# kennethsoh/IE-ACHE

Measured on AMD Instinct MI355X. Metric: bootstrapped gate ops/sec; encrypted 32-bit MUL/sec, higher is better.
Workload: dtype int32; 1 GPU; 16-bit ADD, batch 4096 ciphertext pairs, 1xMI355X (level-batched bootstraps); circuit=add16, batch_per_gpu=4096, bootstraps_per_expr=80, levels=48, params=n=630 N=1024 k=1 l=3 Bgbit=7 ks_t=8 ks_basebit=2, parallelism=batch-sharded x1, kernel=w1x64-radix8-onelimb, overlap_streams=2, rccl_ranks=0

## Files before the change

ie-ache_amd/csrc/blind_rotate_w64.hip:

```cpp
#include "blind_rotate_w64.h"

#include <cstdio>
#include <algorithm>
#include <stdexcept>
#include <type_traits>
#include <vector>

#include "br_step.h"
#include "mix_plan.h"

namespace ieache {
namespace w64 {

using namespace dev;

namespace {

__global__ __launch_bounds__(64) void k_bk_to_spectrum_w64(const Torus32* bk_raw, double2* bkf) {
    __shared__ __align__(16) double2 sT[kTile];
    __shared__ __align__(16) double2 sTw[kTwElems];
    const int lane = threadIdx.x;
    build_twiddles(sTw, lane, 64);
    __syncthreads();
    const LaneRoots R = make_roots(sTw, lane);
    const size_t poly = blockIdx.x;
    const Torus32* src = bk_raw + poly * kN;
    const size_t irow = poly >> 1, c = poly & 1;
#pragma unroll 1
    for (int limb = 0; limb < 2; limb++) {
        double2 x[8];
#pragma unroll
        for (int r = 0; r < 8; r++) {
            const int32_t v0 = src[64 * r + lane], v1 = src[64 * r + lane + kM];
            const int32_t lo0 = (int16_t)(v0 & 0xFFFF), lo1 = (int16_t)(v1 & 0xFFFF);
            const int32_t e0 = limb ? (int32_t)(((int64_t)v0 - lo0) >> 16) : lo0;
            const int32_t e1 = limb ? (int32_t)(((int64_t)v1 - lo1) >> 16) : lo1;
            x[r] = make_double2((double)e0, (double)e1);
        }
        fft512_forward<true>(x, sT, lane, R);
        double2* dst = bkf + ((irow * 4 + c * 2 + limb) * 8) * 64 + lane;
#pragma unroll
        for (int k2 = 0; k2 < 8; k2++) dst[k2 * 64] = x[k2];
    }
}

__global__ __launch_bounds__(64) void k_bk_to_spectrum_w64_1(const Torus32* bk_raw, double2* bkf1) {
    __shared__ __align__(16) double2 sT[kTile];
    __shared__ __align__(16) double2 sTw[kTwElems];
    const int lane = threadIdx.x;
    build_twiddles(sTw, lane, 64);
    __syncthreads();
    const LaneRoots R = make_roots(sTw, lane);
    const size_t poly = blockIdx.x;
    const Torus32* src = bk_raw + poly * kN;
    double2 x[8];
#pragma unroll
    for (int r = 0; r < 8; r++) {
        const double2 v = make_double2((double)src[64 * r + lane], (double)src[64 * r + lane + kM]);
        x[r] = v;
    }
    fft512_forward<true>(x, sT, lane, R);
    double2* dst = bkf1 + (poly * 8) * 64 + lane;
#pragma unroll
    for (int k2 = 0; k2 < 8; k2++) dst[k2 * 64] = x[k2];
}

template <bool TV>
__global__ __launch_bounds__(128) void k_br_prologue(DevKeys K, WorkDesc W, uint16_t* st_bara, int32_t nb, int32_t* st_acc) {
    __shared__ int32_t s_barb;
    const int tid = threadIdx.x;
    const int32_t n = K.n;
    const int64_t item = (int64_t)blockIdx.x;
    const GateInst g = resolve(W, W.item0 + item, K.stride);
    uint16_t* bara = st_bara + (size_t)item * nb;
    for (int32_t i = tid; i <= n; i += 128) {
        const int32_t bar = modswitch2N(combined_coef(g, i, n), 11);
        if (i < n)
            bara[i] = (uint16_t)bar;
        else
            s_barb = bar;
    }
    __syncthreads();
    const int32_t a0 = (2 * kN - s_barb) & (2 * kN - 1);
    int32_t* acc = st_acc + (size_t)item * 2 * kN;
    const Torus32* v = TV ? test_poly_row(W, W.item0 + item, kN) : nullptr;
#pragma unroll
    for (int r = 0; r < 8; r++) {
        const int32_t j = 128 * r + tid;
        acc[j] = 0;
        if (TV)
            acc[kN + j] = rot_coef(v, j, a0, kN);
        else
            acc[kN + j] = ((j - a0) & (2 * kN - 1)) < kN ? kMU : -kMU;
    }
}

template <int L, int BGBIT, int XLANE = 1>
__global__ __launch_bounds__(128, 2) void k_blind_rotate_w2(DevKeys K, const double2* __restrict__ bkf,
                                                           const uint16_t* __restrict__ st_bara, int32_t nb,
                                                           int32_t* st_acc, int32_t i0, int32_t i1, Torus32* ext,
                                                           const double2* __restrict__ gtw) {
    extern __shared__ __align__(16) unsigned char smem[];
    double2* sT_all = reinterpret_cast<double2*>(smem);
    double2* sTw = sT_all + 2 * kTile;
    int32_t* acc = reinterpret_cast<int32_t*>(sTw + kTwElems);
    const int tid = threadIdx.x, lane = tid & 63, wave = tid >> 6;
    double2* sT = sT_all + wave * kTile;
    const double2* sTp = sT_all + (wave ^ 1) * kTile;
    const int64_t item = (int64_t)blockIdx.x;
    const uint16_t* __restrict__ bara = st_bara + (size_t)item * nb;
    int32_t* gacc = st_acc + (size_t)item * 2 * kN;
    load_twiddles(sTw, gtw, tid, 128);
    const LaneRoots R = make_roots(sTw, lane);
    copy_acc<128>(acc, gacc, tid);
    __syncthreads();

    uint32_t dec_offset = decomposition_offset<L, BGBIT>();
    int32_t* accw = acc + wave * kN;

    const int32_t my_a = lane_amounts(bara, i0, i1, lane);
#pragma unroll 1
    for (int32_t i = i0; i < i1; i++) {
        const int32_t a = __builtin_amdgcn_readlane(my_a, i - i0);
        if (a == 0) continue;
        const double2* __restrict__ bki = bkf + (size_t)i * (2 * L * 4 * kM) + (size_t)(2 * wave) * kM + lane;
        double2 s[2][8];
        uint32_t v0[8], v1[8];
#pragma unroll
        for (int r = 0; r < 8; r++) {
            const int32_t j = 64 * r + lane;
            v0[r] = (((uint32_t)rot_coef(accw, j, a, kN) - (uint32_t)accw[j]) + dec_offset) ^ dec_offset;
            v1[r] = (((uint32_t)rot_coef(accw, j + kM, a, kN) - (uint32_t)accw[j + kM]) + dec_offset) ^ dec_offset;
        }
        auto digit_row = [&](const int q, auto first) {
            constexpr bool FIRST = decltype(first)::value;
            const int sh = 32 - (q + 1) * BGBIT;
            const double2* __restrict__ bown = bki + (size_t)(wave * L + q) * (4 * kM);
            const double2* __restrict__ bpar = bki + (size_t)((wave ^ 1) * L + q) * (4 * kM);
            double2 x[8];
            digits_to_double2<BGBIT>(x, v0, v1, sh);
            double2 bA[8], bB[8], bC[8];
#pragma unroll
            for (int k = 0; k < 8; k++) bA[k] = bown[k * 64];
            __builtin_amdgcn_sched_barrier(0);
            fft512_forward<true, XLANE>(x, sT, lane, R);
#pragma unroll
            for (int k = 0; k < 8; k++) sT[k * 64 + lane] = x[k];
#pragma unroll
            for (int k = 0; k < 8; k++) bB[k] = bown[(8 + k) * 64];
#pragma unroll
            for (int k = 0; k < 8; k++) bC[k] = bpar[k * 64];
            __builtin_amdgcn_sched_barrier(0);
            mac_row<FIRST>(s[0], x, bA);
            __builtin_amdgcn_sched_barrier(0);
#pragma unroll
            for (int k = 0; k < 8; k++) bA[k] = bpar[(8 + k) * 64];
            __builtin_amdgcn_sched_barrier(0);
            mac_row<FIRST>(s[1], x, bB);
            __syncthreads();
#pragma unroll
            for (int k = 0; k < 8; k++) x[k] = sTp[k * 64 + lane];
            mac_row<false>(s[0], x, bC);
            mac_row<false>(s[1], x, bA);
            __syncthreads();
        };
        digit_row(0, std::true_type{});
#pragma unroll 1
        for (int q = 1; q < L; q++) digit_row(q, std::false_type{});
        fft512_inverse_pair<true>(s[0], s[1], sT, lane, R);
#pragma unroll
        for (int r = 0; r < 8; r++) {
            double unused = 0.0;
            const uint32_t l0 = round_coef(s[0][r].x, untwist_gain(r), false, unused), l1 = round_coef(s[0][r].y, untwist_gain(r), false, unused);
            const uint32_t h0 = round_coef(s[1][r].x, untwist_gain(r), false, unused), h1 = round_coef(s[1][r].y, untwist_gain(r), false, unused);
            const int32_t j = 64 * r + lane;
            accw[j] = (int32_t)((uint32_t)accw[j] + l0 + (h0 << 16));
            accw[j + kM] = (int32_t)((uint32_t)accw[j + kM] + l1 + (h1 << 16));
        }
    }
    __syncthreads();
    finish_slice<128>(ext, item, acc, gacc, tid);
}


template <int L, int BGBIT, int GUARD, bool DIAG = false, int G = kW1Gates>
__global__ __launch_bounds__(64 * G, 2) void k_blind_rotate_w1b(DevKeys K, const double2* __restrict__ bkf1,
                                                                       const uint16_t* __restrict__ st_bara, int32_t nb,
                                                                       int32_t* st_acc, int64_t items, int32_t i0, int32_t i1,
                                                                       Torus32* ext, unsigned* guard,
                                                                       const double2* __restrict__ gtw, unsigned long long* diag = nullptr) {
    extern __shared__ __align__(16) unsigned char smem[];
    int32_t* acc_all = reinterpret_cast<int32_t*>(smem);
    double2* sT_all = reinterpret_cast<double2*>(smem + (size_t)G * 2 * kN * 4);
    double2* sTw = sT_all + G * kTile;
    const int tid = threadIdx.x, lane = tid & 63;
    const int wave = __builtin_amdgcn_readfirstlane(tid >> 6);
    double2* sT = sT_all + wave * kTile;
    int32_t* acc = acc_all + wave * 2 * kN;
    const int64_t item = (int64_t)blockIdx.x * G + wave;
    load_twiddles(sTw, gtw, tid, 64 * G);
    __syncthreads();
    if (item >= items) return;
    const LaneRoots R = make_roots(sTw, lane);
    const uint16_t* __restrict__ bara = st_bara + (size_t)item * nb;
    int32_t* gacc = st_acc + (size_t)item * 2 * kN;
    {
        const int4* src = reinterpret_cast<const int4*>(gacc);
        int4* dst = reinterpret_cast<int4*>(acc);
#pragma unroll
        for (int r = 0; r < 8; r++) dst[64 * r + lane] = src[64 * r + lane];
    }
    wave_sync();

    constexpr uint32_t halfBg = 1u << (BGBIT - 1);
    uint32_t dec_offset = 0;
#pragma unroll
    for (int q = 1; q <= L; q++) dec_offset += halfBg << (32 - q * BGBIT);
    double dev_max = 0.0;
    constexpr int kRowBytes = 2 * kM * (int)sizeof(double2), kStepBytes = 2 * L * kRowBytes;
    const __amdgpu_buffer_rsrc_t bk_rsrc = bk_resource(bkf1, K.n, kStepBytes);
    const int lane16 = bk_lane_offset(lane);
    const unsigned char* accb = reinterpret_cast<const unsigned char*>(acc_all);
    const uint32_t pb0 = (uint32_t)wave * (2 * kN * 4);

    unsigned long long tsum[8] = {0, 0, 0, 0, 0, 0, 0, 0}, tlast = 0;
    if (DIAG) tlast = stamp();
    const int32_t my_a = lane_amounts(bara, i0, i1, lane);
#pragma unroll 1
    for (int32_t i = i0; i < i1; i++) {
        const int32_t a = __builtin_amdgcn_readlane(my_a, i - i0);
        if (a == 0) continue;
        const int bki = i * kStepBytes;
        double2 s[2][8];
        uint32_t v0[8], v1[8];
        const uint32_t jb4 = ((uint32_t)(lane - a) & (2 * kN - 1)) << 2;
        auto decompose = [&](const uint32_t pb) {
            const int32_t* accp = reinterpret_cast<const int32_t*>(accb + pb);
            decompose_rotated(v0, v1, accb, accp, pb, jb4, lane, dec_offset);
        };
        auto digit_row = [&](const int sh, const int brow, auto first) {
            constexpr bool FIRST = decltype(first)::value;
            double2 x[8], bA[8], bB[8];
            load_bk_block(bA, bk_rsrc, lane16, brow);
            digits_to_double2<BGBIT>(x, v0, v1, sh);
            __builtin_amdgcn_sched_barrier(0);
            stamp_phase<DIAG>(tsum, tlast, 1);
            fft512_forward<true, 1>(x, sT, lane, R);
            stamp_phase<DIAG>(tsum, tlast, 2);
            load_bk_block(bB, bk_rsrc, lane16, brow + kRowBytes / 2);
            __builtin_amdgcn_sched_barrier(0);
#pragma unroll
            for (int k = 0; k < 8; k++) s[0][k] = mac<FIRST>(s[0][k], x[k], bA[k]);
#pragma unroll
            for (int k = 0; k < 8; k++) s[1][k] = mac<FIRST>(s[1][k], x[k], bB[k]);
            stamp_phase<DIAG>(tsum, tlast, 3);
        };
        decompose(pb0);
        stamp_phase<DIAG>(tsum, tlast, 0);
        digit_row(32 - BGBIT, bki, std::true_type{});
#pragma unroll 1
        for (int row = 1; row < L; row++) digit_row(32 - (row + 1) * BGBIT, bki + row * kRowBytes, std::false_type{});
        decompose(pb0 + 4096u);
        stamp_phase<DIAG>(tsum, tlast, 0);
#pragma unroll 1
        for (int row = L; row < 2 * L; row++) digit_row(32 - (row - L + 1) * BGBIT, bki + row * kRowBytes, std::false_type{});
        fft512_inverse_pair<true>(s[0], s[1], sT, lane, R);
        stamp_phase<DIAG>(tsum, tlast, 4);
#pragma unroll
        for (int c = 0; c < 2; c++) {
            uint32_t* accc = reinterpret_cast<uint32_t*>(acc) + c * kN;
#pragma unroll
            for (int r = 0; r < 8; r++) {
                const bool watched = GUARD == 1 || (GUARD == 2 && (r & 3) == 0);
                const uint32_t d0 = round_coef(s[c][r].x, untwist_gain(r), watched, dev_max), d1 = round_coef(s[c][r].y, untwist_gain(r), watched, dev_max);
                const int32_t j = 64 * r + lane;
                __hip_atomic_fetch_add(&accc[j], d0, __ATOMIC_RELAXED, __HIP_MEMORY_SCOPE_WAVEFRONT);
                __hip_atomic_fetch_add(&accc[j + kM], d1, __ATOMIC_RELAXED, __HIP_MEMORY_SCOPE_WAVEFRONT);
            }
        }
        wave_sync();
        stamp_phase<DIAG>(tsum, tlast, 5);
    }
    if (DIAG && diag && lane == 0) {
#pragma unroll
        for (int t = 0; t < 8; t++) atomicAdd(&diag[(wave & 1) * 8 + t], tsum[t]);
    }
    if (GUARD) publish_guard(dev_max, guard, lane);
    finish_slice<64>(ext, item, acc, gacc, lane);
}

template <int L, int BGBIT, int G = kW1Gates>
__global__ __launch_bounds__(64 * G, 2) void k_blind_rotate_x1(DevKeys K, const double2* __restrict__ bkf,
                                                                      const uint16_t* __restrict__ st_bara, int32_t nb,
                                                                      int32_t* st_acc, int64_t items, int32_t i0, int32_t i1,
                                                                      Torus32* ext, const double2* __restrict__ gtw) {
    extern __shared__ __align__(16) unsigned char smem[];
    int32_t* acc_all = reinterpret_cast<int32_t*>(smem);
    double2* sT_all = reinterpret_cast<double2*>(smem + (size_t)G * 2 * kN * 4);
    double2* sTw = sT_all + G * kTile;
    const int tid = threadIdx.x, lane = tid & 63;
    const int wave = __builtin_amdgcn_readfirstlane(tid >> 6);
    double2* sT = sT_all + wave * kTile;
    int32_t* acc = acc_all + wave * 2 * kN;
    const int64_t item = (int64_t)blockIdx.x * G + wave;
    load_twiddles(sTw, gtw, tid, 64 * G);
    __syncthreads();
    if (item >= items) return;
    const LaneRoots R = make_roots(sTw, lane);
    const uint16_t* __restrict__ bara = st_bara + (size_t)item * nb;
    int32_t* gacc = st_acc + (size_t)item * 2 * kN;
    {
        const int4* src = reinterpret_cast<const int4*>(gacc);
        int4* dst = reinterpret_cast<int4*>(acc);
#pragma unroll
        for (int r = 0; r < 8; r++) dst[64 * r + lane] = src[64 * r + lane];
    }
    wave_sync();

    constexpr uint32_t halfBg = 1u << (BGBIT - 1);
    uint32_t dec_offset = 0;
#pragma unroll
    for (int q = 1; q <= L; q++) dec_offset += halfBg << (32 - q * BGBIT);
    constexpr int kBlockBytes = kM * (int)sizeof(double2), kRowBytes = 4 * kBlockBytes, kStepBytes = 2 * L * kRowBytes;
    const __amdgpu_buffer_rsrc_t bk_rsrc = bk_resource(bkf, K.n, kStepBytes);
    const int lane16 = bk_lane_offset(lane);
    const unsigned char* accb = reinterpret_cast<const unsigned char*>(acc_all);
    const uint32_t pb0 = (uint32_t)wave * (2 * kN * 4);

    const int32_t my_a = lane_amounts(bara, i0, i1, lane);
#pragma unroll 1
    for (int32_t i = i0; i < i1; i++) {
        const int32_t a = __builtin_amdgcn_readlane(my_a, i - i0);
        if (a == 0) continue;
        const int bki = i * kStepBytes;
        double2 s[4][8];
        uint32_t v0[8], v1[8];
        const uint32_t jb4 = ((uint32_t)(lane - a) & (2 * kN - 1)) << 2;
        auto decompose = [&](const uint32_t pb, const uint32_t jb) {
            const int32_t* accp = reinterpret_cast<const int32_t*>(accb + pb);
            decompose_rotated(v0, v1, accb, accp, pb, jb, lane, dec_offset);
        };
        auto digit_row = [&](const int sh, const int brow, auto first) {
            constexpr bool FIRST = decltype(first)::value;
            double2 x[8], bA[8], bB[8];
            digits_to_double2<BGBIT>(x, v0, v1, sh);
            __builtin_amdgcn_sched_barrier(0);
            auto req = [&]() { load_bk_block(bA, bk_rsrc, lane16, brow); };
            fft512_forward<true, 1, decltype(req), true>(x, sT, lane, R, req);
            load_bk_block(bB, bk_rsrc, lane16, brow + kBlockBytes);
            __builtin_amdgcn_sched_barrier(0);
            mac_row<FIRST>(s[0], x, bA);
            __builtin_amdgcn_sched_barrier(0);
            load_bk_block(bA, bk_rsrc, lane16, brow + 2 * kBlockBytes);
            __builtin_amdgcn_sched_barrier(0);
            mac_row<FIRST>(s[1], x, bB);
            __builtin_amdgcn_sched_barrier(0);
            load_bk_block(bB, bk_rsrc, lane16, brow + 3 * kBlockBytes);
            __builtin_amdgcn_sched_barrier(0);
            mac_row<FIRST>(s[2], x, bA);
            mac_row<FIRST>(s[3], x, bB);
        };
        decompose(pb0, jb4);
        digit_row(32 - BGBIT, bki, std::true_type{});
#pragma unroll 1
        for (int row = 1; row < L; row++) digit_row(32 - (row + 1) * BGBIT, bki + row * kRowBytes, std::false_type{});
        uint32_t jb4b = jb4;
        asm volatile("" : "+v"(jb4b));
        decompose(pb0 + 4096u, jb4b);
#pragma unroll 1
        for (int row = L; row < 2 * L; row++) digit_row(32 - (row - L + 1) * BGBIT, bki + row * kRowBytes, std::false_type{});
#pragma unroll
        for (int c = 0; c < 2; c++) {
            fft512_inverse_pair<true>(s[2 * c], s[2 * c + 1], sT, lane, R);
            uint32_t* accc = reinterpret_cast<uint32_t*>(acc) + c * kN;
#pragma unroll
            for (int r = 0; r < 8; r++) {
                double unused = 0.0;
                const uint32_t d0 = round_coef(s[2 * c][r].x, untwist_gain(r), false, unused) + (round_coef(s[2 * c + 1][r].x, untwist_gain(r), false, unused) << 16);
                const uint32_t d1 = round_coef(s[2 * c][r].y, untwist_gain(r), false, unused) + (round_coef(s[2 * c + 1][r].y, untwist_gain(r), false, unused) << 16);
                const int32_t j = 64 * r + lane;
                __hip_atomic_fetch_add(&accc[j], d0, __ATOMIC_RELAXED, __HIP_MEMORY_SCOPE_WAVEFRONT);
                __hip_atomic_fetch_add(&accc[j + kM], d1, __ATOMIC_RELAXED, __HIP_MEMORY_SCOPE_WAVEFRONT);
            }
        }
        wave_sync();
    }
    finish_slice<64>(ext, item, acc, gacc, lane);
}

template <int L, int BGBIT, int GUARD>
__global__ __launch_bounds__(128, 2) void k_blind_rotate_w2r(DevKeys K, const double2* __restrict__ bkf1,
                                                            const uint16_t* __restrict__ st_bara, int32_t nb,
                                                            int32_t* st_acc, int32_t i0, int32_t i1, Torus32* ext,
                                                            unsigned* guard, const double2* __restrict__ gtw) {
    extern __shared__ __align__(16) unsigned char smem[];
    int32_t* acc = reinterpret_cast<int32_t*>(smem);
    double2* sT_all = reinterpret_cast<double2*>(smem + (size_t)2 * kN * 4);
    double2* sTw = sT_all + 2 * kTile;
    const int tid = threadIdx.x, lane = tid & 63;
    const int wave = __builtin_amdgcn_readfirstlane(tid >> 6);
    double2* sT = sT_all + wave * kTile;
    const double2* sTp = sT_all + (wave ^ 1) * kTile;
    const int64_t item = (int64_t)blockIdx.x;
    const uint16_t* __restrict__ bara = st_bara + (size_t)item * nb;
    int32_t* gacc = st_acc + (size_t)item * 2 * kN;
    load_twiddles(sTw, gtw, tid, 128);
    const LaneRoots R = make_roots(sTw, lane);
    {
        const int4* src = reinterpret_cast<const int4*>(gacc);
        int4* dst = reinterpret_cast<int4*>(acc);
#pragma unroll
        for (int r = 0; r < 4; r++) dst[128 * r + tid] = src[128 * r + tid];
    }
    __syncthreads();

    constexpr uint32_t halfBg = 1u << (BGBIT - 1);
    uint32_t dec_offset = 0;
#pragma unroll
    for (int q = 1; q <= L; q++) dec_offset += halfBg << (32 - q * BGBIT);
    double dev_max = 0.0;
    constexpr int kRowBytes = 2 * kM * (int)sizeof(double2), kStepBytes = 2 * L * kRowBytes;
    const __amdgpu_buffer_rsrc_t bk_rsrc = bk_resource(bkf1, K.n, kStepBytes);
    const int lane16 = bk_lane_offset(lane);
    const unsigned char* accb = reinterpret_cast<const unsigned char*>(acc);
    const uint32_t pb = (uint32_t)wave * (kN * 4);
    const int32_t* accp = acc + wave * kN;
    uint32_t* accu = reinterpret_cast<uint32_t*>(acc) + wave * kN;

    int32_t my_a = 0;
#pragma unroll 1
    for (int32_t i = i0; i < i1; i++) {
        if (((i - i0) & 63) == 0) my_a = (i + lane < i1) ? (int32_t)bara[i + lane] : 0;
        const int32_t a = __builtin_amdgcn_readlane(my_a, (i - i0) & 63);
        if (a == 0) continue;
        const int bki = i * kStepBytes + wave * L * kRowBytes;
        double2 s[2][8];
        uint32_t v0[8], v1[8];
        const uint32_t jb4 = ((uint32_t)(lane - a) & (2 * kN - 1)) << 2;
#pragma unroll
        for (int r = 0; r < 8; r++) {
            const uint32_t t = jb4 + 256u * r;
            const uint32_t o0 = (t & 4092u) | pb, o1 = o0 ^ 2048u;
            const int32_t m0 = __builtin_amdgcn_sbfe((int32_t)t, 12, 1), m1 = __builtin_amdgcn_sbfe((int32_t)(t + 2048u), 12, 1);
            const uint32_t rv0 = *reinterpret_cast<const uint32_t*>(accb + o0), rv1 = *reinterpret_cast<const uint32_t*>(accb + o1);
            const uint32_t pv0 = (uint32_t)accp[64 * r + lane], pv1 = (uint32_t)accp[64 * r + lane + kM];
            v0[r] = ((rv0 ^ (uint32_t)m0) + ((dec_offset - pv0) - (uint32_t)m0)) ^ dec_offset;
            v1[r] = ((rv1 ^ (uint32_t)m1) + ((dec_offset - pv1) - (uint32_t)m1)) ^ dec_offset;
        }
        auto digit_row = [&](const int sh, const int brow, auto first) {
            constexpr bool FIRST = decltype(first)::value;
            double2 x[8], bA[8], bB[8];
            load_bk_block(bA, bk_rsrc, lane16, brow);
            digits_to_double2<BGBIT>(x, v0, v1, sh);
            __builtin_amdgcn_sched_barrier(0);
            fft512_forward<true, 1>(x, sT, lane, R);
            load_bk_block(bB, bk_rsrc, lane16, brow + kRowBytes / 2);
            __builtin_amdgcn_sched_barrier(0);
#pragma unroll
            for (int k = 0; k < 8; k++) s[0][k] = mac<FIRST>(s[0][k], x[k], bA[k]);
#pragma unroll
            for (int k = 0; k < 8; k++) s[1][k] = mac<FIRST>(s[1][k], x[k], bB[k]);
        };
        digit_row(32 - BGBIT, bki, std::true_type{});
#pragma unroll 1
        for (int q = 1; q < L; q++) digit_row(32 - (q + 1) * BGBIT, bki + q * kRowBytes, std::false_type{});
        double2 y[8];
#pragma unroll
        for (int k = 0; k < 8; k++) {
            const double2 mine = wave ? s[1][k] : s[0][k], theirs = wave ? s[0][k] : s[1][k];
            sT[k * 64 + lane] = theirs;
            y[k] = mine;
        }
        __syncthreads();
#pragma unroll
        for (int k = 0; k < 8; k++) {
            const double2 z = sTp[k * 64 + lane];
            y[k] = cadd(y[k], z);
        }
        __syncthreads();
        fft512_inverse<true>(y, sT, lane, R);
#pragma unroll
        for (int r = 0; r < 8; r++) {
            const bool watched = GUARD == 1 || (GUARD == 2 && (r & 3) == 0);
            const uint32_t d0 = round_coef(y[r].x, untwist_gain(r), watched, dev_max), d1 = round_coef(y[r].y, untwist_gain(r), watched, dev_max);
            const int32_t j = 64 * r + lane;
            __hip_atomic_fetch_add(&accu[j], d0, __ATOMIC_RELAXED, __HIP_MEMORY_SCOPE_WAVEFRONT);
            __hip_atomic_fetch_add(&accu[j + kM], d1, __ATOMIC_RELAXED, __HIP_MEMORY_SCOPE_WAVEFRONT);
        }
        wave_sync();
    }
    __syncthreads();
    if (GUARD) publish_guard(dev_max, guard, lane);
    finish_slice<128>(ext, item, acc, gacc, tid);
}

template <int L, int BGBIT, int GUARD>
__global__ __launch_bounds__(256, 2) void k_blind_rotate_w4r(DevKeys K, const double2* __restrict__ bkf1,
                                                            const uint16_t* __restrict__ st_bara, int32_t nb,
                                                            int32_t* st_acc, int32_t i0, int32_t i1, Torus32* ext,
                                                            unsigned* guard, const double2* __restrict__ gtw, int32_t flip_period) {
    extern __shared__ __align__(16) unsigned char smem[];
    int32_t* acc = reinterpret_cast<int32_t*>(smem);
    double2* sT_all = reinterpret_cast<double2*>(smem + (size_t)2 * kN * 4);
    double2* sX = sT_all + 4 * kTile;
    double2* sTw = sX + 2 * 8 * 64;
    const int tid = threadIdx.x, lane = tid & 63;
    const int wave = __builtin_amdgcn_readfirstlane(tid >> 6) ^ (int)((blockIdx.x / (unsigned)flip_period) & 1u);
    const int pol = wave >> 1;
    const bool light = wave & 1;
    double2* sT = sT_all + wave * kTile;
    const int64_t item = (int64_t)blockIdx.x;
    const uint16_t* __restrict__ bara = st_bara + (size_t)item * nb;
    int32_t* gacc = st_acc + (size_t)item * 2 * kN;
    load_twiddles(sTw, gtw, tid, 256);
    const LaneRoots R = make_roots(sTw, lane);
    {
        const int4* src = reinterpret_cast<const int4*>(gacc);
        int4* dst = reinterpret_cast<int4*>(acc);
#pragma unroll
        for (int r = 0; r < 2; r++) dst[256 * r + tid] = src[256 * r + tid];
    }
    __syncthreads();

    constexpr uint32_t halfBg = 1u << (BGBIT - 1);
    uint32_t dec_offset = 0;
#pragma unroll
    for (int q = 1; q <= L; q++) dec_offset += halfBg << (32 - q * BGBIT);
    double dev_max = 0.0;
    constexpr int kRowBytes = 2 * kM * (int)sizeof(double2), kStepBytes = 2 * L * kRowBytes;
    const __amdgpu_buffer_rsrc_t bk_rsrc = bk_resource(bkf1, K.n, kStepBytes);
    const int lane16 = bk_lane_offset(lane);
    const unsigned char* accb = reinterpret_cast<const unsigned char*>(acc);
    const uint32_t pb = (uint32_t)pol * (kN * 4);
    const int32_t* accp = acc + pol * kN;
    uint32_t* accu = reinterpret_cast<uint32_t*>(acc) + pol * kN;
    const int q0 = light ? L - 1 : 0, q1 = light ? L : (L > 1 ? L - 1 : 1);
    double2* slot_extra = sX + pol * (8 * 64);
    const double2* in_a = light ? (pol == 0 ? sT_all + 0 * kTile : sX + 0 * (8 * 64)) : nullptr;
    const double2* in_b = light ? (pol == 0 ? sX + 1 * (8 * 64) : sT_all + 1 * kTile) : nullptr;
    const double2* in_c = light ? (pol == 0 ? sT_all + 3 * kTile : sT_all + 2 * kTile) : nullptr;
    double2* scratch = sT_all + (pol == 0 ? 0 : 2) * kTile;

    int32_t my_a = 0;
#pragma unroll 1
    for (int32_t i = i0; i < i1; i++) {
        if (((i - i0) & 63) == 0) my_a = (i + lane < i1) ? (int32_t)bara[i + lane] : 0;
        const int32_t a = __builtin_amdgcn_readlane(my_a, (i - i0) & 63);
        if (a == 0) continue;
        const int bki = i * kStepBytes + pol * L * kRowBytes;
        double2 s[2][8];
        uint32_t v0[8], v1[8];
        const uint32_t jb4 = ((uint32_t)(lane - a) & (2 * kN - 1)) << 2;
        decompose_rotated(v0, v1, accb, accp, pb, jb4, lane, dec_offset);
        auto digit_row = [&](const int sh, const int brow, auto first) {
            constexpr bool FIRST = decltype(first)::value;
            double2 x[8], bA[8], bB[8];
            load_bk_block(bA, bk_rsrc, lane16, brow);
            digits_to_double2<BGBIT>(x, v0, v1, sh);
            __builtin_amdgcn_sched_barrier(0);
            fft512_forward<true, 1>(x, sT, lane, R);
            load_bk_block(bB, bk_rsrc, lane16, brow + kRowBytes / 2);
            __builtin_amdgcn_sched_barrier(0);
#pragma unroll
            for (int k = 0; k < 8; k++) s[0][k] = mac<FIRST>(s[0][k], x[k], bA[k]);
#pragma unroll
            for (int k = 0; k < 8; k++) s[1][k] = mac<FIRST>(s[1][k], x[k], bB[k]);
        };
        digit_row(32 - (q0 + 1) * BGBIT, bki + q0 * kRowBytes, std::true_type{});
#pragma unroll 1
        for (int q = q0 + 1; q < q1; q++) digit_row(32 - (q + 1) * BGBIT, bki + q * kRowBytes, std::false_type{});
        double2 y[8];
#pragma unroll
        for (int k = 0; k < 8; k++) {
            const double2 own = pol ? s[1][k] : s[0][k], other = pol ? s[0][k] : s[1][k];
            if (light) {
                y[k] = own;
                sT[k * 64 + lane] = other;
            } else {
                sT[k * 64 + lane] = own;
                slot_extra[k * 64 + lane] = other;
            }
        }
        __syncthreads();
        if (light) {
#pragma unroll
            for (int k = 0; k < 8; k++) {
                const double2 za = in_a[k * 64 + lane], zb = in_b[k * 64 + lane], zc = in_c[k * 64 + lane];
                y[k] = cadd(cadd(y[k], za), cadd(zb, zc));
            }
            fft512_inverse<true>(y, scratch, lane, R);
#pragma unroll
// ... 599 lines not shown
```

ie-ache_amd/csrc/fft512.h:

```cpp
#pragma once
#include <hip/hip_runtime.h>

#include <cstdint>
#include <type_traits>

#include "dft8_twist.h"

namespace ieache {
namespace w64 {
namespace {

constexpr int kN = 1024, kM = 512;

__device__ __forceinline__ double2 cadd(double2 a, double2 b) { return make_double2(a.x + b.x, a.y + b.y); }
__device__ __forceinline__ double2 csub(double2 a, double2 b) { return make_double2(a.x - b.x, a.y - b.y); }
template <bool INV>
__device__ __forceinline__ double2 rot90(double2 z) {
    return INV ? make_double2(-z.y, z.x) : make_double2(z.y, -z.x);
}
template <bool CONJ>
__device__ __forceinline__ double2 cmulx(double2 a, double2 b) {
    return CONJ ? make_double2(fma(a.x, b.x, a.y * b.y), fma(a.y, b.x, -a.x * b.y))
                : make_double2(fma(a.x, b.x, -a.y * b.y), fma(a.x, b.y, a.y * b.x));
}

template <bool INV>
__device__ __forceinline__ void dft8(double2 (&x)[8]) {
    const double2 a0 = cadd(x[0], x[4]), a1 = cadd(x[1], x[5]), a2 = cadd(x[2], x[6]), a3 = cadd(x[3], x[7]);
    const double2 b0 = csub(x[0], x[4]), t1 = csub(x[1], x[5]), t2 = csub(x[2], x[6]), t3 = csub(x[3], x[7]);
    const double2 c0 = cadd(a0, a2), c1 = cadd(a1, a3), c2 = csub(a0, a2), c3 = rot90<INV>(csub(a1, a3));
    x[0] = cadd(c0, c1);
    x[4] = csub(c0, c1);
    x[2] = cadd(c2, c3);
    x[6] = csub(c2, c3);
    const double2 b2 = rot90<INV>(t2);
    const double2 b1 = INV ? make_double2(t1.x - t1.y, t1.x + t1.y) : make_double2(t1.x + t1.y, t1.y - t1.x);
    const double2 b3 = INV ? make_double2(-t3.x - t3.y, t3.x - t3.y) : make_double2(t3.y - t3.x, -t3.x - t3.y);
    const double2 e0 = cadd(b0, b2), e2 = csub(b0, b2);
    const double2 s = cadd(b1, b3), d = rot90<INV>(csub(b1, b3));
    x[1] = make_double2(fma(kR, s.x, e0.x), fma(kR, s.y, e0.y));
    x[5] = make_double2(fma(-kR, s.x, e0.x), fma(-kR, s.y, e0.y));
    x[3] = make_double2(fma(kR, d.x, e2.x), fma(kR, d.y, e2.y));
    x[7] = make_double2(fma(-kR, d.x, e2.x), fma(-kR, d.y, e2.y));
}

__device__ __forceinline__ void wave_sync() {
    __builtin_amdgcn_fence(__ATOMIC_RELEASE, "wavefront");
    __builtin_amdgcn_wave_barrier();
    __builtin_amdgcn_fence(__ATOMIC_ACQUIRE, "wavefront");
}

__device__ __forceinline__ unsigned long long stamp() {
    __builtin_amdgcn_sched_barrier(0);
    unsigned long long t;
    asm volatile("s_memtime %0\n\ts_waitcnt lgkmcnt(0)" : "=s"(t)::"memory");
    __builtin_amdgcn_sched_barrier(0);
    return t;
}

template <bool WSYNC>
__device__ __forceinline__ void tile_sync() {
    if (WSYNC)
        wave_sync();
    else
        __syncthreads();
    __builtin_amdgcn_sched_barrier(0);
}

constexpr int kTwElems = 8 * 64 + 8 * 8;
struct LaneRoots {
    const double2* t1;
    const double2* t2;
    __device__ __forceinline__ double2 a(int k) const { return t1[k * 64]; }
    __device__ __forceinline__ double2 b(int k) const { return t2[k * 8]; }
};
__device__ __forceinline__ void build_twiddles(double2* tw, int tid, int nthreads) {
    double s, c;
    for (int idx = tid; idx < 512; idx += nthreads) {
        const int k = idx >> 6, lane = idx & 63;
        sincospi((double)(lane * (1 - 4 * k)) / 1024.0, &s, &c);
        tw[idx] = make_double2(c, s);
    }
    for (int idx = tid; idx < 64; idx += nthreads) {
        const int k = idx >> 3, p0 = idx & 7;
        sincospi(-(double)(p0 * k) / 32.0, &s, &c);
        tw[512 + idx] = make_double2(c, s);
    }
}

__global__ __launch_bounds__(128) void k_build_twiddle_table(double2* tw) { build_twiddles(tw, threadIdx.x, 128); }

__device__ __forceinline__ void load_twiddles(double2* sTw, const double2* __restrict__ gtw, int tid, int nthreads) {
    for (int idx = tid; idx < kTwElems; idx += nthreads) sTw[idx] = gtw[idx];
}

__device__ __forceinline__ LaneRoots make_roots(const double2* tw, int lane) {
    LaneRoots r;
    r.t1 = tw + lane;
    r.t2 = tw + 512 + (lane & 7);
    return r;
}

typedef unsigned v2u_t __attribute__((ext_vector_type(2)));

template <int B>
__device__ __forceinline__ void swap_dwords(unsigned& lo, unsigned& hi) {
    static_assert(B == 5 || B == 4, "v_permlane32_swap / v_permlane16_swap");
    const v2u_t r = B == 5 ? __builtin_amdgcn_permlane32_swap(lo, hi, false, false) : __builtin_amdgcn_permlane16_swap(lo, hi, false, false);
    lo = r[0];
    hi = r[1];
}

__device__ __forceinline__ void swap4_row_ror8(unsigned (&a)[4], unsigned (&b)[4]) {
    unsigned na0, na1, na2, na3, nb0, nb1, nb2, nb3;
    asm volatile("s_mov_b32 vcc_lo, 0xff00ff00\n\t"
                 "s_mov_b32 vcc_hi, 0xff00ff00\n\t"
                 "s_nop 1\n\t"
                 "v_cndmask_b32_dpp %4, %8, %12, vcc row_ror:8 row_mask:0xf bank_mask:0xf\n\t"
                 "v_cndmask_b32_dpp %5, %9, %13, vcc row_ror:8 row_mask:0xf bank_mask:0xf\n\t"
                 "v_cndmask_b32_dpp %6, %10, %14, vcc row_ror:8 row_mask:0xf bank_mask:0xf\n\t"
                 "v_cndmask_b32_dpp %7, %11, %15, vcc row_ror:8 row_mask:0xf bank_mask:0xf\n\t"
                 "s_not_b64 vcc, vcc\n\t"
                 "v_cndmask_b32_dpp %0, %12, %8, vcc row_ror:8 row_mask:0xf bank_mask:0xf\n\t"
                 "v_cndmask_b32_dpp %1, %13, %9, vcc row_ror:8 row_mask:0xf bank_mask:0xf\n\t"
                 "v_cndmask_b32_dpp %2, %14, %10, vcc row_ror:8 row_mask:0xf bank_mask:0xf\n\t"
                 "v_cndmask_b32_dpp %3, %15, %11, vcc row_ror:8 row_mask:0xf bank_mask:0xf"
                 : "=&v"(na0), "=&v"(na1), "=&v"(na2), "=&v"(na3), "=&v"(nb0), "=&v"(nb1), "=&v"(nb2), "=&v"(nb3)
                 : "v"(a[0]), "v"(a[1]), "v"(a[2]), "v"(a[3]), "v"(b[0]), "v"(b[1]), "v"(b[2]), "v"(b[3])
                 : "vcc");
    a[0] = na0, a[1] = na1, a[2] = na2, a[3] = na3;
    b[0] = nb0, b[1] = nb1, b[2] = nb2, b[3] = nb3;
}

template <int B>
__device__ __forceinline__ void bitswap(double2 (&x)[8]) {
    constexpr int m = 1 << (B - 3);
#pragma unroll
    for (int r = 0; r < 8; r++) {
        if (r & m) continue;
        unsigned a[4] = {(unsigned)__double2loint(x[r].x), (unsigned)__double2hiint(x[r].x), (unsigned)__double2loint(x[r].y),
                         (unsigned)__double2hiint(x[r].y)};
        unsigned b[4] = {(unsigned)__double2loint(x[r | m].x), (unsigned)__double2hiint(x[r | m].x), (unsigned)__double2loint(x[r | m].y),
                         (unsigned)__double2hiint(x[r | m].y)};
        if constexpr (B == 3) {
            swap4_row_ror8(a, b);
        } else {
#pragma unroll
            for (int q = 0; q < 4; q++) swap_dwords<B>(a[q], b[q]);
        }
        x[r] = make_double2(__hiloint2double((int)a[1], (int)a[0]), __hiloint2double((int)a[3], (int)a[2]));
        x[r | m] = make_double2(__hiloint2double((int)b[1], (int)b[0]), __hiloint2double((int)b[3], (int)b[2]));
    }
}
__device__ __forceinline__ void xlane_hi(double2 (&x)[8]) {
    bitswap<3>(x);
    bitswap<4>(x);
    bitswap<5>(x);
}

constexpr int kTile = 8 * 72;

struct NoHook {
    __device__ __forceinline__ void operator()() const {}
};
template <bool WSYNC, int XLANE = 0, class MID = NoHook, bool MID_LATE = false>
__device__ __forceinline__ void fft512_forward(double2 (&x)[8], double2* sT, int lane, const LaneRoots& R, MID mid = MID()) {
    static_assert(XLANE == 0 || XLANE == 1, "lane-low transposes go through the tile");
    const int hi = lane >> 3, lo = lane & 7;
    const int own = hi * 9 + lo;
    const int blk = hi * 72 + lo;
    double2 tA[8], tB[8];
#pragma unroll
    for (int k = 0; k < 8; k++) tA[k] = R.a(k);
    dft8_twist_fwd(x);
#pragma unroll
    for (int k = 0; k < 8; k++) x[k] = cmulx<false>(x[k], tA[k]);
    if (!std::is_same<MID, NoHook>::value && !MID_LATE) {
        __builtin_amdgcn_sched_barrier(0);
        mid();
        __builtin_amdgcn_sched_barrier(0);
    }
#pragma unroll
    for (int k = 1; k < 8; k++) tB[k] = R.b(k);
    if (XLANE) {
        xlane_hi(x);
    } else {
#pragma unroll
        for (int k0 = 0; k0 < 8; k0++) sT[own + 72 * k0] = x[k0];
        tile_sync<WSYNC>();
#pragma unroll
        for (int p1 = 0; p1 < 8; p1++) x[p1] = sT[blk + 9 * p1];
        tile_sync<WSYNC>();
    }
    dft8<false>(x);
#pragma unroll
    for (int k = 1; k < 8; k++) x[k] = cmulx<false>(x[k], tB[k]);
    if (!std::is_same<MID, NoHook>::value && MID_LATE) {
        __builtin_amdgcn_sched_barrier(0);
        mid();
        __builtin_amdgcn_sched_barrier(0);
    }
#pragma unroll
    for (int k1 = 0; k1 < 8; k1++) sT[blk + 9 * k1] = x[k1];
    tile_sync<WSYNC>();
    const int rd = hi * 72 + lo * 9;
#pragma unroll
    for (int q = 0; q < 8; q++) x[q] = sT[rd + q];
    tile_sync<WSYNC>();
    dft8<false>(x);
}

template <bool WSYNC>
__device__ __forceinline__ void fft512_inverse(double2 (&x)[8], double2* sT, int lane, const LaneRoots& R) {
    const int hi = lane >> 3, lo = lane & 7;
    const int own = hi * 9 + lo, blk = hi * 72 + lo, rd = hi * 72 + lo * 9;
    double2 tA[8], tB[8];
#pragma unroll
    for (int k = 1; k < 8; k++) tB[k] = R.b(k);
    dft8<true>(x);
#pragma unroll
    for (int k = 0; k < 8; k++) tA[k] = R.a(k);
#pragma unroll
    for (int q = 0; q < 8; q++) sT[rd + q] = x[q];
    tile_sync<WSYNC>();
#pragma unroll
    for (int k = 0; k < 8; k++) x[k] = sT[blk + 9 * k];
    tile_sync<WSYNC>();
#pragma unroll
    for (int k = 1; k < 8; k++) x[k] = cmulx<true>(x[k], tB[k]);
    dft8<true>(x);
#pragma unroll
    for (int p1 = 0; p1 < 8; p1++) sT[blk + 9 * p1] = x[p1];
    tile_sync<WSYNC>();
#pragma unroll
    for (int k0 = 0; k0 < 8; k0++) x[k0] = sT[own + 72 * k0];
    tile_sync<WSYNC>();
#pragma unroll
    for (int k = 0; k < 8; k++) x[k] = cmulx<true>(x[k], tA[k]);
    dft8_untwist_inv(x);
}

template <bool WSYNC>
__device__ __forceinline__ void fft512_inverse_pair(double2 (&x)[8], double2 (&y)[8], double2* sT, int lane,
                                                    const LaneRoots& R) {
    const int hi = lane >> 3, lo = lane & 7;
    const int own = hi * 9 + lo, blk = hi * 72 + lo, rd = hi * 72 + lo * 9;
    double2 tA[8], tB[8];
#pragma unroll
    for (int k = 1; k < 8; k++) tB[k] = R.b(k);
    dft8<true>(x);
#pragma unroll
    for (int q = 0; q < 8; q++) sT[rd + q] = x[q];
    tile_sync<WSYNC>();
#pragma unroll
    for (int k = 0; k < 8; k++) x[k] = sT[blk + 9 * k];
    dft8<true>(y);
    __builtin_amdgcn_sched_barrier(0);
#pragma unroll
    for (int k = 0; k < 8; k++) tA[k] = R.a(k);
#pragma unroll
    for (int q = 0; q < 8; q++) sT[rd + q] = y[q];
    tile_sync<WSYNC>();
#pragma unroll
    for (int k = 0; k < 8; k++) y[k] = sT[blk + 9 * k];
#pragma unroll
    for (int k = 1; k < 8; k++) x[k] = cmulx<true>(x[k], tB[k]);
    dft8<true>(x);
    __builtin_amdgcn_sched_barrier(0);
#pragma unroll
    for (int p1 = 0; p1 < 8; p1++) sT[blk + 9 * p1] = x[p1];
    tile_sync<WSYNC>();
#pragma unroll
    for (int k0 = 0; k0 < 8; k0++) x[k0] = sT[own + 72 * k0];
#pragma unroll
    for (int k = 1; k < 8; k++) y[k] = cmulx<true>(y[k], tB[k]);
    dft8<true>(y);
    __builtin_amdgcn_sched_barrier(0);
#pragma unroll
    for (int p1 = 0; p1 < 8; p1++) sT[blk + 9 * p1] = y[p1];
    tile_sync<WSYNC>();
#pragma unroll
    for (int k0 = 0; k0 < 8; k0++) y[k0] = sT[own + 72 * k0];
#pragma unroll
    for (int k = 0; k < 8; k++) x[k] = cmulx<true>(x[k], tA[k]);
    dft8_untwist_inv(x);
    __builtin_amdgcn_sched_barrier(0);
#pragma unroll
    for (int k = 0; k < 8; k++) y[k] = cmulx<true>(y[k], tA[k]);
    dft8_untwist_inv(y);
    tile_sync<WSYNC>();
}

constexpr double kMagic52 = 6755399441055744.0;
__device__ __forceinline__ uint32_t round_coef(double v, double gain, bool watch, double& dev_max) {
    double t;
    if (watch) {
        const double z = v * gain;
        t = z + kMagic52;
        dev_max = fmax(dev_max, fabs(z - (t - kMagic52)));
    } else {
        t = fma(v, gain, kMagic52);
    }
    return (uint32_t)__double2loint(t);
}

typedef int v4i_t __attribute__((ext_vector_type(4)));
__device__ __forceinline__ void load_bk_block(double2 (&dst)[8], __amdgpu_buffer_rsrc_t rsrc, int lane16, int soff) {
#pragma unroll
    for (int k = 0; k < 8; k++) {
        const v4i_t d = __builtin_amdgcn_raw_buffer_load_b128(rsrc, lane16 + (k & 3) * 1024, soff + (k >> 2) * 4096, 0);
        dst[k] = make_double2(__hiloint2double(d.y, d.x), __hiloint2double(d.w, d.z));
    }
}

}
}
}
```

Measured before the change: 214,700 gate ops/s.

## Keep stage-B twiddles in registers and hoist bk load into forward FFT

Adds a ResidentRoots variant that caches six of the second-stage FFT twiddles in registers per lane, so the blind-rotate kernel no longer reloads them from LDS on every FFT. The first bootstrapping-key block load is moved inside the forward FFT through the mid hook, so the global fetch overlaps the first radix-8 stage. The guard deviation tracker becomes a per-step double folded into a float accumulator, and the lane id is pinned through an empty asm to shape register allocation. Together these trade extra VGPRs (roughly 24 for the resident roots) against LDS traffic and exposed load latency, which may lower occupancy under the two-blocks launch bound.

```diff
diff --git a/ie-ache_amd/csrc/blind_rotate_w64.hip b/ie-ache_amd/csrc/blind_rotate_w64.hip
--- a/ie-ache_amd/csrc/blind_rotate_w64.hip
+++ b/ie-ache_amd/csrc/blind_rotate_w64.hip
@@ -201,7 +201,7 @@
     load_twiddles(sTw, gtw, tid, 64 * G);
     __syncthreads();
     if (item >= items) return;
-    const LaneRoots R = make_roots(sTw, lane);
+    const LaneRootsResident R = make_roots<LaneRootsResident>(sTw, lane);
     const uint16_t* __restrict__ bara = st_bara + (size_t)item * nb;
     int32_t* gacc = st_acc + (size_t)item * 2 * kN;
     {
@@ -216,7 +216,7 @@
     uint32_t dec_offset = 0;
 #pragma unroll
     for (int q = 1; q <= L; q++) dec_offset += halfBg << (32 - q * BGBIT);
-    double dev_max = 0.0;
+    float dev_maxf = 0.0f;
     constexpr int kRowBytes = 2 * kM * (int)sizeof(double2), kStepBytes = 2 * L * kRowBytes;
     const __amdgpu_buffer_rsrc_t bk_rsrc = bk_resource(bkf1, K.n, kStepBytes);
     const int lane16 = bk_lane_offset(lane);
@@ -233,6 +233,7 @@
         const int bki = i * kStepBytes;
         double2 s[2][8];
         uint32_t v0[8], v1[8];
+        double dev_max = 0.0;
         const uint32_t jb4 = ((uint32_t)(lane - a) & (2 * kN - 1)) << 2;
         auto decompose = [&](const uint32_t pb) {
             const int32_t* accp = reinterpret_cast<const int32_t*>(accb + pb);
@@ -241,11 +242,11 @@
         auto digit_row = [&](const int sh, const int brow, auto first) {
             constexpr bool FIRST = decltype(first)::value;
             double2 x[8], bA[8], bB[8];
-            load_bk_block(bA, bk_rsrc, lane16, brow);
+            auto request_a = [&]() { load_bk_block(bA, bk_rsrc, lane16, brow); };
             digits_to_double2<BGBIT>(x, v0, v1, sh);
             __builtin_amdgcn_sched_barrier(0);
             stamp_phase<DIAG>(tsum, tlast, 1);
-            fft512_forward<true, 1>(x, sT, lane, R);
+            fft512_forward<true, 1>(x, sT, lane, R, request_a);
             stamp_phase<DIAG>(tsum, tlast, 2);
             load_bk_block(bB, bk_rsrc, lane16, brow + kRowBytes / 2);
             __builtin_amdgcn_sched_barrier(0);
@@ -278,6 +279,7 @@
                 __hip_atomic_fetch_add(&accc[j + kM], d1, __ATOMIC_RELAXED, __HIP_MEMORY_SCOPE_WAVEFRONT);
             }
         }
+        if (GUARD) dev_maxf = fmaxf(dev_maxf, (float)dev_max);
         wave_sync();
         stamp_phase<DIAG>(tsum, tlast, 5);
     }
@@ -285,8 +287,10 @@
 #pragma unroll
         for (int t = 0; t < 8; t++) atomicAdd(&diag[(wave & 1) * 8 + t], tsum[t]);
     }
-    if (GUARD) publish_guard(dev_max, guard, lane);
-    finish_slice<64>(ext, item, acc, gacc, lane);
+    int elane = lane;
+    asm volatile("" : "+v"(elane));
+    if (GUARD) publish_guard((double)dev_maxf, guard, elane);
+    finish_slice<64>(ext, item, acc, gacc, elane);
 }
 
 template <int L, int BGBIT, int G = kW1Gates>
diff --git a/ie-ache_amd/csrc/fft512.h b/ie-ache_amd/csrc/fft512.h
--- a/ie-ache_amd/csrc/fft512.h
+++ b/ie-ache_amd/csrc/fft512.h
@@ -5,6 +5,7 @@
 #include <type_traits>
 
 #include "dft8_twist.h"
+#include "tw_roots.h"
 
 namespace ieache {
 namespace w64 {
@@ -67,13 +68,8 @@
     __builtin_amdgcn_sched_barrier(0);
 }
 
-constexpr int kTwElems = 8 * 64 + 8 * 8;
-struct LaneRoots {
-    const double2* t1;
-    const double2* t2;
-    __device__ __forceinline__ double2 a(int k) const { return t1[k * 64]; }
-    __device__ __forceinline__ double2 b(int k) const { return t2[k * 8]; }
-};
+using LaneRoots = TableRoots<double2>;
+using LaneRootsResident = ResidentRoots<double2, 6>;
 __device__ __forceinline__ void build_twiddles(double2* tw, int tid, int nthreads) {
     double s, c;
     for (int idx = tid; idx < 512; idx += nthreads) {
@@ -94,10 +90,10 @@
     for (int idx = tid; idx < kTwElems; idx += nthreads) sTw[idx] = gtw[idx];
 }
 
-__device__ __forceinline__ LaneRoots make_roots(const double2* tw, int lane) {
-    LaneRoots r;
-    r.t1 = tw + lane;
-    r.t2 = tw + 512 + (lane & 7);
+template <class ROOTS = LaneRoots>
+__device__ __forceinline__ ROOTS make_roots(const double2* tw, int lane) {
+    ROOTS r;
+    r.init(tw, lane);
     return r;
 }
 
@@ -163,8 +159,8 @@
 struct NoHook {
     __device__ __forceinline__ void operator()() const {}
 };
-template <bool WSYNC, int XLANE = 0, class MID = NoHook, bool MID_LATE = false>
-__device__ __forceinline__ void fft512_forward(double2 (&x)[8], double2* sT, int lane, const LaneRoots& R, MID mid = MID()) {
+template <bool WSYNC, int XLANE = 0, class MID = NoHook, bool MID_LATE = false, class ROOTS = LaneRoots>
+__device__ __forceinline__ void fft512_forward(double2 (&x)[8], double2* sT, int lane, const ROOTS& R, MID mid = MID()) {
     static_assert(XLANE == 0 || XLANE == 1, "lane-low transposes go through the tile");
     const int hi = lane >> 3, lo = lane & 7;
     const int own = hi * 9 + lo;
@@ -210,8 +206,8 @@
     dft8<false>(x);
 }
 
-template <bool WSYNC>
-__device__ __forceinline__ void fft512_inverse(double2 (&x)[8], double2* sT, int lane, const LaneRoots& R) {
+template <bool WSYNC, class ROOTS = LaneRoots>
+__device__ __forceinline__ void fft512_inverse(double2 (&x)[8], double2* sT, int lane, const ROOTS& R) {
     const int hi = lane >> 3, lo = lane & 7;
     const int own = hi * 9 + lo, blk = hi * 72 + lo, rd = hi * 72 + lo * 9;
     double2 tA[8], tB[8];
@@ -240,9 +236,9 @@
     dft8_untwist_inv(x);
 }
 
-template <bool WSYNC>
+template <bool WSYNC, class ROOTS = LaneRoots>
 __device__ __forceinline__ void fft512_inverse_pair(double2 (&x)[8], double2 (&y)[8], double2* sT, int lane,
-                                                    const LaneRoots& R) {
+                                                    const ROOTS& R) {
     const int hi = lane >> 3, lo = lane & 7;
     const int own = hi * 9 + lo, blk = hi * 72 + lo, rd = hi * 72 + lo * 9;
     double2 tA[8], tB[8];
diff --git a/ie-ache_amd/csrc/tw_roots.h b/ie-ache_amd/csrc/tw_roots.h
--- /dev/null
+++ b/ie-ache_amd/csrc/tw_roots.h
@@ -0,0 +1,46 @@
+#pragma once
+
+#ifndef IEACHE_HD
+#ifdef __HIPCC__
+#define IEACHE_HD __device__ __forceinline__
+#else
+#define IEACHE_HD inline
+#endif
+#endif
+
+namespace ieache {
+namespace w64 {
+
+constexpr int kTwElems = 8 * 64 + 8 * 8;
+template <class V>
+IEACHE_HD const V* tw_a_base(const V* tw, int lane) { return tw + lane; }
+template <class V>
+IEACHE_HD const V* tw_b_base(const V* tw, int lane) { return tw + 512 + (lane & 7); }
+
+template <class V>
+struct TableRoots {
+    const V* t1;
+    const V* t2;
+    IEACHE_HD V a(int k) const { return t1[k * 64]; }
+    IEACHE_HD V b(int k) const { return t2[k * 8]; }
+    IEACHE_HD void init(const V* tw, int lane) {
+        t1 = tw_a_base(tw, lane);
+        t2 = tw_b_base(tw, lane);
+    }
+};
+
+template <class V, int NRES = 7>
+struct ResidentRoots {
+    TableRoots<V> table;
+    V tb[8];
+    IEACHE_HD V a(int k) const { return table.a(k); }
+    IEACHE_HD V b(int k) const { return k <= NRES ? tb[k] : table.b(k); }
+    IEACHE_HD void init(const V* tw, int lane) {
+        table.init(tw, lane);
+#pragma unroll
+        for (int k = 1; k <= NRES; k++) tb[k] = table.b(k);
+    }
+};
+
+}
+}
```

Result: faster. 217,900 gate ops/s (median of 6 runs) (+1.5%).
